# ucla-vision/xivo

Measured on AMD Instinct MI355X. Metric: EKF updates/sec (state dim 250, 80 feats) @1 GPU; % MFMA roofline, higher is better.
Workload: dtype f64; 1 GPU; MH gating + UpdateJosephForm: state dim 250, 80 features (M=160), XIVO row sparsity, P/H/inn/R resident in HBM; filters_per_gpu=16384, global_batch=16384, parallelism=replicas x1 (no collective), pipeline=sparse-H (row-pair compressed H, whitened in-solve Joseph form), hand_over=dense H -> row-pair compressed rows every step, inside the timed region, route=sparse_in_solve, not_spd_filters=0

## Files before the change

### include/xivo_hip.h

```cpp
#ifndef XIVO_HIP_H_
#define XIVO_HIP_H_

#include <stddef.h>

#ifdef __cplusplus
extern "C" {
#endif

typedef struct xivo_hip_ctx xivo_hip_ctx;

enum {
  XIVO_HIP_OK = 0,
  XIVO_HIP_ERR_INVALID = -1,
  XIVO_HIP_ERR_HIP = -2,
  XIVO_HIP_ERR_NOT_SPD = -3,
  XIVO_HIP_ERR_NOMEM = -4,
  XIVO_HIP_ERR_UNSUPPORTED = -5,
  XIVO_HIP_ERR_FULL = -6
};

enum {
  XIVO_HIP_FLAG_NONE = 0u,
  XIVO_HIP_FLAG_FIX_GROUP_BLOCK = 1u,
  XIVO_HIP_FLAG_PROFILE = 2u,
// ... 29 lines not shown
  double Rbc[9], Tbc[3];
  double Vsb[3], bg[3], ba[3];
  double Rsg[9];
} xivo_pose_in;

typedef struct {
  double Rsb[9], Tsb[3];
} xivo_group_in;

typedef struct {
  double x[3];
  double xp[2];
  int ref_sind;
  int sind;
} xivo_feat_in;

#define XIVO_OOS_MAX_OBS 16
typedef struct {
  double Xs[3];
  int n_obs;
  int group_sind[XIVO_OOS_MAX_OBS];
  double xp[XIVO_OOS_MAX_OBS][2];
} xivo_oos_in;

int xivo_hip_create(xivo_hip_ctx** out, int device, int N, int M_max, int batch_max, unsigned flags);
void xivo_hip_destroy(xivo_hip_ctx* ctx);
const char* xivo_hip_strerror(int status);
int xivo_hip_sync(xivo_hip_ctx* ctx);
int xivo_hip_device_count(void);
int xivo_hip_device_numa_node(int device);
int xivo_hip_set_flags(xivo_hip_ctx* ctx, unsigned flags);

int xivo_hip_upload_P(xivo_hip_ctx* ctx, int b0, int nb, const double* P, long stride, int ld);
int xivo_hip_download_P(xivo_hip_ctx* ctx, int b0, int nb, double* P, long stride, int ld);
int xivo_hip_snapshot_P(xivo_hip_ctx* ctx);
int xivo_hip_restore_P(xivo_hip_ctx* ctx);
int xivo_hip_p_zero_rc(xivo_hip_ctx* ctx, int b, int off, int len);
int xivo_hip_p_copy_rc(xivo_hip_ctx* ctx, int b, int dst, int src, int len);
int xivo_hip_p_set_block3(xivo_hip_ctx* ctx, int b, int off, const double* P3);
int xivo_hip_p_diag(xivo_hip_ctx* ctx, int b, double* diag_out);

int xivo_hip_set_measurements(xivo_hip_ctx* ctx, int b0, int nb, int M,
                              const double* H, long strideH, int ldh,
                              const double* inn, long strideInn,
                              const double* diagR, long strideR);
int xivo_hip_set_measurements_device(xivo_hip_ctx* ctx, int b0, int nb, int M,
                                     const double* dH, long strideH, int ldh,
                                     const double* dInn, long strideInn,
                                     const double* dR, long strideR);
int xivo_hip_update_joseph(xivo_hip_ctx* ctx, int B);
int xivo_hip_get_err(xivo_hip_ctx* ctx, int b0, int nb, double* err, long stride);
int xivo_hip_get_status(xivo_hip_ctx* ctx, int b0, int nb, int* status);
int xivo_hip_get_ldlt_used(xivo_hip_ctx* ctx, int b0, int nb, int* used);
#define XIVO_HIP_HOST_P_RESIDENT 1u
#define XIVO_HIP_HOST_KEEP_P 2u
int xivo_hip_update_joseph_host(xivo_hip_ctx* ctx, int b, int M, const double* H, int ldh, const double* inn,
                                const double* diagR, double* P, int ldp, double* err_out, unsigned mode);
int xivo_hip_selftest_fused_tiles(int column_blocks, int* per_simd);
int xivo_hip_selftest_fused_shape(int Mp, int Np, int pw, char* label, int n);
int xivo_hip_selftest_host_compress(const double* H, int ldh, int M, int N, int pairs_clear, int* idx, double* val, int* nc, int* pw);
#define XIVO_HIP_LAUNCH_GATE 0
#define XIVO_HIP_LAUNCH_OOS_COMPRESS 1
#define XIVO_HIP_LAUNCH_PROP_TAIL 2
int xivo_hip_selftest_glevel_launch(int kind, int a, int b, int c, char* label, int n);
int xivo_hip_selftest_ctx_allocs(xivo_hip_ctx* ctx, int* live, unsigned long long* bytes);
int xivo_hip_mh_gate_dense(xivo_hip_ctx* ctx, int B, int F, double R, double mh_thresh,
                           double mh_mult, int min_inliers,
                           unsigned char* inlier_mask_out, double* mh_dist_out);

int xivo_hip_update_dense_gated(xivo_hip_ctx* ctx, int B, int F, double R, double mh_thresh,
                                double mh_mult, int min_inliers);
int xivo_hip_get_gate(xivo_hip_ctx* ctx, int B, int F, unsigned char* inlier_mask_out, double* mh_dist_out);

int xivo_hip_set_layout(xivo_hip_ctx* ctx, const xivo_layout* layout, const xivo_cam* cam);
int xivo_hip_set_scene(xivo_hip_ctx* ctx, int b0, int nb, int F,
                       const xivo_pose_in* poses, const xivo_group_in* groups ,
                       const xivo_feat_in* feats );
int xivo_hip_jacobians_instate(xivo_hip_ctx* ctx, int B);
int xivo_hip_get_jacobians(xivo_hip_ctx* ctx, int b0, int nb, double* J2x21, double* inn2);
typedef struct {
  int td;
  int Cg;
  int cam_begin;
  int cam_dim;
} xivo_calib_layout;
typedef struct {
  double gyro[3];
  double Cg[9];
  double td;
  double Ca[9];
  double intr[9];
} xivo_calib_in;
int xivo_hip_set_calib(xivo_hip_ctx* ctx, const xivo_calib_layout* layout);
int xivo_hip_set_calib_state(xivo_hip_ctx* ctx, int b0, int nb, const xivo_calib_in* calib );
int xivo_hip_get_calib_state(xivo_hip_ctx* ctx, int b0, int nb, xivo_calib_in* calib_out );
int xivo_hip_set_calib_gyro(xivo_hip_ctx* ctx, int b0, int nb, const double* gyro3);
int xivo_hip_get_jacobians_calib(xivo_hip_ctx* ctx, int b0, int nb, double* Jc2x22);
int xivo_hip_mh_gate(xivo_hip_ctx* ctx, int B, double R, double mh_thresh, double mh_mult,
                     int min_inliers, unsigned char* inlier_mask_out, double* mh_dist_out);
int xivo_hip_stack(xivo_hip_ctx* ctx, int B, double R);
int xivo_hip_oos_project(xivo_hip_ctx* ctx, int b0, int nb, int n_oos, const xivo_oos_in* feats,
                         double Roos, int* rows_out);
#define XIVO_HIP_OOS_WHOLE_BUFFER 1u
int xivo_hip_oos_project_ex(xivo_hip_ctx* ctx, int b0, int nb, int n_oos, const xivo_oos_in* feats,
                            double Roos, int* rows_out, unsigned options);
typedef struct {
// ... 190 lines not shown
```

### xivo_amd/csrc/capi_update.hip

```cpp
#include <algorithm>

#include "capi_internal.h"

using namespace xivo_hip;
using namespace xivo_hip::capi;

namespace {

enum UpdateRoute : int { ROUTE_FUSED = 0, ROUTE_SPARSE_IN_SOLVE, ROUTE_SPARSE_WHITENED, ROUTE_SPARSE_SYMMETRIC, ROUTE_SPARSE_TAIL,
                         ROUTE_DENSE_ASCODED, ROUTE_DENSE_WHITENED, ROUTE_DENSE_SYMMETRIC, ROUTE_COUNT };
static const char* kRouteNames[ROUTE_COUNT] = {"fused", "sparse_in_solve", "sparse_whitened", "sparse_symmetric", "sparse_tail",
                                               "dense_ascoded", "dense_whitened", "dense_symmetric"};
struct UpdatePlan {
  int route;
  bool sparse;
  bool in_solve;
  bool latency;
  bool stream8;
  bool f32_whitened;
};

static UpdatePlan plan_update(const xivo_hip_ctx* c, int b0, int B, bool gate) {
  const StagedRows& r = c->rows;
  const int Np = c->Np, Mp = r.rows_padded();
// ... 514 lines not shown
int xivo_hip_update_dense_gated(xivo_hip_ctx* c, int B, int F, double R, double mh_thresh, double mh_mult,
                                int min_inliers) {
  if (c && hipSetDevice(c->device) != hipSuccess) return XIVO_HIP_ERR_HIP;
  if (!c || B <= 0 || B > c->Bmax || c->rows.rows_padded() <= 0 || F <= 0 || 2 * F > c->rows.rows()) return XIVO_HIP_ERR_INVALID;
  int rc = ensure_gate_buffers(c, F);
  if (rc) return rc;
  GateParams gp{F, R, mh_thresh, mh_mult, min_inliers};
  return update_chunks(c, B, F > min_inliers ? &gp : nullptr);
}

int xivo_hip_last_path(xivo_hip_ctx* c) { return c ? c->last_path : -1; }
int xivo_hip_last_route(xivo_hip_ctx* c) { return c ? c->last_route : -1; }
const char* xivo_hip_route_name(int route) { return route >= 0 && route < ROUTE_COUNT ? kRouteNames[route] : ""; }

double xivo_hip_stage_bytes(xivo_hip_ctx* c, int stage) {
  return (c && stage >= 0 && stage < ST_COUNT) ? c->stage_bytes[stage] : 0.0;
}

const char* xivo_hip_stage_kernel(xivo_hip_ctx* c, int stage) {
  return (c && stage >= 0 && stage < ST_COUNT) ? c->stage_kernel[stage] : "";
}

int xivo_hip_get_gate(xivo_hip_ctx* c, int B, int F, unsigned char* mask_out, double* dist_out) {
  if (c && hipSetDevice(c->device) != hipSuccess) return XIVO_HIP_ERR_HIP;
  if (!c || B <= 0 || B > c->Bmax || F <= 0 || !c->mask) return XIVO_HIP_ERR_INVALID;
  const bool strided = c->rows.gate_layout() == GateLayout::strided;
  const size_t ld = strided ? (size_t)c->Fmax : (size_t)F;
  if (strided && F != c->F) return XIVO_HIP_ERR_INVALID;
  if (mask_out) { int rc = d2h_rows(c, mask_out, F, c->mask, ld, F, B); if (rc) return rc; }
  if (dist_out) {
    int rc = d2h_rows(c, dist_out, F * sizeof(double), c->dist, ld * sizeof(double), F * sizeof(double), B);
    if (rc) return rc;
  }
  return XIVO_HIP_OK;
}

int xivo_hip_get_err(xivo_hip_ctx* c, int b0, int nb, double* err, long stride) {
  if (c && hipSetDevice(c->device) != hipSuccess) return XIVO_HIP_ERR_HIP;
  if (bad_range(c, b0, nb) || !err || stride < c->N) return XIVO_HIP_ERR_INVALID;
  if (nb == 0) return XIVO_HIP_OK;
  return d2h_rows(c, err, (size_t)stride * sizeof(double), c->err.from(b0).p, (size_t)c->err.stride * sizeof(double),
                  (size_t)c->N * sizeof(double), nb);
}

int xivo_hip_get_ldlt_used(xivo_hip_ctx* c, int b0, int nb, int* used) {
  if (c && hipSetDevice(c->device) != hipSuccess) return XIVO_HIP_ERR_HIP;
  if (bad_range(c, b0, nb) || !used) return XIVO_HIP_ERR_INVALID;
  if (nb == 0) return XIVO_HIP_OK;
  HIP_TRY(hipMemcpyAsync(used, c->ldlt_used + b0, (size_t)nb * sizeof(int), hipMemcpyDeviceToHost, c->stream));
  HIP_TRY(hipStreamSynchronize(c->stream));
  return XIVO_HIP_OK;
}

int xivo_hip_get_status(xivo_hip_ctx* c, int b0, int nb, int* status) {
  if (c && hipSetDevice(c->device) != hipSuccess) return XIVO_HIP_ERR_HIP;
  if (bad_range(c, b0, nb) || !status) return XIVO_HIP_ERR_INVALID;
  if (nb == 0) return XIVO_HIP_OK;
  HIP_TRY(hipMemcpyAsync(status, c->status + b0, (size_t)nb * sizeof(int), hipMemcpyDeviceToHost, c->stream));
  HIP_TRY(hipStreamSynchronize(c->stream));
  for (int i = 0; i < nb; ++i) if (status[i]) return XIVO_HIP_ERR_NOT_SPD;
  return XIVO_HIP_OK;
}

int xivo_hip_selftest_fused_tiles(int column_blocks, int* per_simd) { return fused_tiles_selftest(column_blocks, per_simd); }
int xivo_hip_selftest_fused_shape(int Mp, int Np, int pw, char* label, int n) {
  return fused_shape_selftest(Mp, Np, pw, label, n > 0 ? (size_t)n : 0);
}

int xivo_hip_selftest_host_compress(const double* H, int ldh, int M, int N, int pairs_clear, int* idx, double* val, int* nc, int* pw) {
  if (!H || !idx || !val || !nc || !pw || M <= 0 || N <= 0 || ldh < M || 2 * pairs_clear < M) return XIVO_HIP_ERR_INVALID;
  xivo_hip_ctx::HostCompressScratch sc;
  return host_compress(sc, H, ldh, M, N, pairs_clear, idx, val, nc, pw);
}

int xivo_hip_update_joseph_host(xivo_hip_ctx* c, int b, int M, const double* H, int ldh, const double* inn,
                                const double* diagR, double* P, int ldp, double* err_out, unsigned mode) {
  if (c && hipSetDevice(c->device) != hipSuccess) return XIVO_HIP_ERR_HIP;
  const bool p_up = !(mode & XIVO_HIP_HOST_P_RESIDENT), p_down = !(mode & XIVO_HIP_HOST_KEEP_P);
  if (bad_range(c, b, 1) || !H || !inn || !diagR || !err_out || M <= 0 || M > c->Mmax || ldh < M ||
      ((p_up || p_down) && (!P || ldp < c->N)))
    return XIVO_HIP_ERR_INVALID;
  const int N = c->N, Np = c->Np, pairs_clear = c->Mpmax / 2;
  auto al = [](size_t x) { return (x + 63) & ~(size_t)63; };
  const size_t o_idx = 0, o_val = al(o_idx + (size_t)pairs_clear * ELL_W * sizeof(int)),
               o_inn = al(o_val + (size_t)pairs_clear * ELL_W * 2 * sizeof(double)), o_R = al(o_inn + (size_t)c->Mpmax * sizeof(double)),
               o_flags = al(o_R + (size_t)c->Mpmax * sizeof(double)), o_Pin = al(o_flags + 4 * sizeof(int)),
               o_Pout = al(o_Pin + (size_t)N * N * sizeof(double)), o_err = al(o_Pout + (size_t)N * N * sizeof(double)),
               o_st = al(o_err + (size_t)N * sizeof(double)), total = al(o_st + 4 * sizeof(int));
  if (!c->pin_h) {
    if (hipHostMalloc(reinterpret_cast<void**>(&c->pin_h), total, hipHostMallocMapped) != hipSuccess) { c->pin_h = nullptr; (void)hipGetLastError(); return XIVO_HIP_ERR_NOMEM; }
    if (hipHostGetDevicePointer(reinterpret_cast<void**>(&c->pin_d), c->pin_h, 0) != hipSuccess || !c->pin_d) {
      hipHostFree(c->pin_h); c->pin_h = nullptr; c->pin_d = nullptr; (void)hipGetLastError(); return XIVO_HIP_ERR_HIP;
    }
  }
  int nc = 0, pw = 0, over = 1;
  const bool want_ell = !(c->flags & XIVO_HIP_FLAG_DENSE_H) && meas_compress_fits(c->Mpmax, Np);
  if (want_ell)
    over = host_compress(c->hc, H, ldh, M, N, pairs_clear, reinterpret_cast<int*>(c->pin_h + o_idx),
                         reinterpret_cast<double*>(c->pin_h + o_val), &nc, &pw);
  if (over) {
    int rc = XIVO_HIP_OK;
    if (p_up) rc = xivo_hip_upload_P(c, b, 1, P, (long)ldp * N, ldp);
    if (!rc) rc = xivo_hip_set_measurements(c, b, 1, M, H, (long)ldh * N, ldh, inn, M, diagR, M);
    if (!rc) rc = update_joseph_range(c, b, 1);
    if (rc) return rc;
    int st = 0;
// ... 68 lines not shown
```

### xivo_amd/csrc/chol_f64.hip

```cpp
#include <stdlib.h>
#include <stdio.h>

#include "mfma_util.h"
#include "chol_device.h"
#include "gate_device.h"

namespace xivo_hip {

namespace {


__global__ __launch_bounds__(64, 4) void chol_f64_kernel(CholArgs g) {
  const int filt = blockIdx.x;
  if (filt >= g.batch) return;
  double* S = g.S + (long)filt * g.strideS;
  double* invD = g.invD + (long)filt * g.strideInvD;
  const long ld = g.lds;
  const int nb = g.Mp / 16;
  const int lane = threadIdx.x;
  const int li = lane & 15, lg = lane >> 4;

  __shared__ double sInv[2][256];
  int bad = 0;

  for (int j = 0; j < nb; ++j) {
    {
      d4 acc0 = d4{0.0, 0.0, 0.0, 0.0}, acc1 = d4{0.0, 0.0, 0.0, 0.0};
      for (int k = 0; k < j; ++k) {
        const double a0 = S[(16 * j + li) + (long)(16 * k + 0 + lg) * ld];
        const double a1 = S[(16 * j + li) + (long)(16 * k + 4 + lg) * ld];
        const double a2 = S[(16 * j + li) + (long)(16 * k + 8 + lg) * ld];
        const double a3 = S[(16 * j + li) + (long)(16 * k + 12 + lg) * ld];
        acc0 = mfma(a0, a0, acc0);
        acc1 = mfma(a1, a1, acc1);
        acc0 = mfma(a2, a2, acc0);
        acc1 = mfma(a3, a3, acc1);
      }
      d4 x, y;
#pragma unroll
      for (int r = 0; r < 4; ++r) x[r] = S[(16 * j + li) + (long)(16 * j + lg + 4 * r) * ld] - (acc0[r] + acc1[r]);
      factor_invert_diag(x, y, bad, 16 * j, li, lg);
#pragma unroll
      for (int r = 0; r < 4; ++r) {
        const int c = lg + 4 * r;
        if (c <= li) {
          S[(16 * j + li) + (long)(16 * j + c) * ld] = x[r];
          S[(16 * j + c) + (long)(16 * j + li) * ld] = x[r];
        }
        sInv[0][c + li * 16] = y[r];
        sInv[1][li + c * 16] = y[r];
      }
    }
    __syncthreads();
    for (int e = lane; e < 512; e += 64) invD[(long)j * 512 + e] = (&sInv[0][0])[e];

    for (int i = j + 1; i < nb; i += 2) {
      const bool two = (i + 1 < nb);
      const int i2 = two ? i + 1 : i;
      d4 accA = d4{0.0, 0.0, 0.0, 0.0}, accB = d4{0.0, 0.0, 0.0, 0.0};
      d4 accA1 = d4{0.0, 0.0, 0.0, 0.0}, accB1 = d4{0.0, 0.0, 0.0, 0.0};
      for (int k = 0; k < j; ++k) {
#pragma unroll
        for (int s = 0; s < 4; ++s) {
          const long col = (long)(16 * k + 4 * s + lg) * ld;
          const double a = S[(16 * j + li) + col];
          const double b1 = S[(16 * i + li) + col];
          const double b2 = S[(16 * i2 + li) + col];
          if (s & 1) { accA1 = mfma(a, b1, accA1); accB1 = mfma(a, b2, accB1); }
          else { accA = mfma(a, b1, accA); accB = mfma(a, b2, accB); }
        }
      }
      d4 rhsA, rhsB;
#pragma unroll
      for (int r = 0; r < 4; ++r) {
        rhsA[r] = S[(16 * i + li) + (long)(16 * j + lg + 4 * r) * ld] - (accA[r] + accA1[r]);
        rhsB[r] = S[(16 * i2 + li) + (long)(16 * j + lg + 4 * r) * ld] - (accB[r] + accB1[r]);
      }
      d4 outA = d4{0.0, 0.0, 0.0, 0.0}, outB = d4{0.0, 0.0, 0.0, 0.0};
#pragma unroll
      for (int s = 0; s < 4; ++s) {
        const double iv = sInv[0][li + (4 * s + lg) * 16];
        outA = mfma(iv, rhsA[s], outA);
        outB = mfma(iv, rhsB[s], outB);
      }
#pragma unroll
      for (int r = 0; r < 4; ++r) {
        S[(16 * i + li) + (long)(16 * j + lg + 4 * r) * ld] = outA[r];
        S[(16 * j + lg + 4 * r) + (long)(16 * i + li) * ld] = outA[r];
        if (two) {
          S[(16 * i2 + li) + (long)(16 * j + lg + 4 * r) * ld] = outB[r];
          S[(16 * j + lg + 4 * r) + (long)(16 * i2 + li) * ld] = outB[r];
        }
      }
    }
    __syncthreads();
  }
  if (lane == 0) g.status[filt] = bad;
}


template <int NB, int MINB, bool PRE, bool UPFRONT, int NW = 4, bool GATE = false>
__global__ __launch_bounds__(64 * NW, MINB) void chol_reg_f64_kernel(CholArgs g, int mirror, CholGateArgs gt) {
  constexpr int RW = (NB + NW - 1) / NW;
  const int filt = blockIdx.x;
  if (filt >= g.batch) return;
  double* S = g.S + (long)filt * g.strideS;
  double* invD = g.invD + (long)filt * g.strideInvD;
  const long ld = g.lds;
  const int nb = g.Mp / 16;
  const int tid = threadIdx.x, lane = tid & 63, wave = __builtin_amdgcn_readfirstlane(tid >> 6);
  const int li = lane & 15, lg = lane >> 4;

  __shared__ double sInv[2][256];
  __shared__ __attribute__((aligned(16))) double sRow[(NB - 1) * 256];
  __shared__ int sBad;
  if (tid == 0) sBad = 0;
  __shared__ unsigned char sRej[GATE ? 16 * NB : 1];
  if constexpr (GATE) {
    static_assert(NW == 4 && !UPFRONT, "the gate rides in the many-factors instantiations");
    double* sdist = sRow;
    const int F = gt.F;
    double* inn = gt.inn + (long)filt * gt.strideInn;
    double* dr = gt.diagR + (long)filt * gt.strideR;
    const double* sd = gt.Sdiag + (long)filt * gt.strideSdiag;
    for (int f = tid; f < F; f += 64 * NW) {
      const double s00 = sd[4 * f] - dr[2 * f] + gt.R;
      const double s10 = sd[4 * f + 2];
      const double s11 = sd[4 * f + 3] - dr[2 * f + 1] + gt.R;
      sdist[f] = mh_dist_2x2(s00, s10, s11, inn[2 * f], inn[2 * f + 1]);
    }
    for (int m = tid; m < 16 * NB; m += 64 * NW) sRej[m] = 0;
    __syncthreads();
    if (wave == 0) {
      const double th = relax_threshold(sdist, F, gt.thresh, gt.mult, gt.min_inliers, lane);
      if (lane == 0) sdist[F] = th;
    }
    __syncthreads();
    const double th = sdist[F];
    for (int f = tid; f < F; f += 64 * NW) {
      const bool in = sdist[f] < th;
      gt.mask[(long)filt * F + f] = in ? 1 : 0;
      gt.dist[(long)filt * F + f] = sdist[f];
      if (!in) {
        sRej[2 * f] = 1; sRej[2 * f + 1] = 1;
        inn[2 * f] = 0.0; inn[2 * f + 1] = 0.0;
        dr[2 * f] = 1.0; dr[2 * f + 1] = 1.0;
        double* val = gt.ellval + (long)filt * gt.strideVal + (long)f * gt.ell_w * 2;
        for (int t = 0; t < 2 * gt.ell_w; ++t) val[t] = 0.0;
      }
    }
    __syncthreads();
    double* PHT = gt.PHT + (long)filt * gt.stridePHT;
    for (int f = 0; f < F; ++f) {
      if (!sRej[2 * f]) continue;
      for (int n = tid; n < gt.Np; n += 64 * NW) { PHT[n + (long)(2 * f) * gt.ldpht] = 0.0; PHT[n + (long)(2 * f + 1) * gt.ldpht] = 0.0; }
    }
    __syncthreads();
  }
  auto gated = [&](double v, int row, int col) -> double {
    if constexpr (GATE) return (sRej[row] | sRej[col]) ? (row == col ? 1.0 : 0.0) : v;
    else return v;
  };

  d4 L[RW][NB];
  d4 sdiag[RW];
#pragma unroll
  for (int ii = 0; ii < RW; ++ii) {
    const int jd = wave + NW * ii;
    if (NW == 4 && jd < nb) {
#pragma unroll
      for (int r = 0; r < 4; ++r) sdiag[ii][r] = gated(S[(16 * jd + li) + (long)(16 * jd + lg + 4 * r) * ld], 16 * jd + li, 16 * jd + lg + 4 * r);
    }
  }

  if (UPFRONT) {
#pragma unroll
    for (int ii = 0; ii < RW; ++ii) {
      const int i = wave + NW * ii;
#pragma unroll
      for (int k = 0; k < NB; ++k) {
        if (k < NW * ii + NW - 1 && k < i && i < nb) {
#pragma unroll
          for (int r = 0; r < 4; ++r) L[ii][k][r] = S[(16 * i + li) + (long)(16 * k + lg + 4 * r) * ld];
        }
      }
    }
  }
  d4 pre0 = d4{0.0, 0.0, 0.0, 0.0}, pre1 = d4{0.0, 0.0, 0.0, 0.0};
  static_for<NB>([&](auto jc) {
    constexpr int j = decltype(jc)::value;
    if (j < nb) {
    constexpr int owner = j % NW, jj = j / NW;
    d4 sreg[RW];
#pragma unroll
    for (int ii = 0; ii < RW; ++ii) {
      const int i = wave + NW * ii;
      if (!UPFRONT && NW * ii + NW - 1 > j && i > j && i < nb) {
#pragma unroll
        for (int r = 0; r < 4; ++r) sreg[ii][r] = gated(S[(16 * i + li) + (long)(16 * j + lg + 4 * r) * ld], 16 * i + li, 16 * j + lg + 4 * r);
      }
    }
    d4 x;
    if (NW != 4 && wave == owner) {
#pragma unroll
      for (int r = 0; r < 4; ++r) sdiag[jj][r] = S[(16 * j + li) + (long)(16 * j + lg + 4 * r) * ld];
    }
    if (wave == owner) {
      d4 acc0 = d4{0.0, 0.0, 0.0, 0.0}, acc1 = d4{0.0, 0.0, 0.0, 0.0};
      if (PRE) { acc0 = pre0; acc1 = pre1; }
#pragma unroll
      for (int k = (PRE && j > 0) ? j - 1 : 0; k < j; ++k) {
        const d4 a = L[jj][k];
        acc0 = mfma(a[0], a[0], acc0);
        acc1 = mfma(a[1], a[1], acc1);
        acc0 = mfma(a[2], a[2], acc0);
        acc1 = mfma(a[3], a[3], acc1);
      }
#pragma unroll
      for (int r = 0; r < 4; ++r) x[r] = sdiag[jj][r] - (acc0[r] + acc1[r]);
    }
    if constexpr (PRE && j + 1 < NB) if (j + 1 < nb && wave == ((j + 1) % NW)) {
      pre0 = d4{0.0, 0.0, 0.0, 0.0}; pre1 = d4{0.0, 0.0, 0.0, 0.0};
#pragma unroll
      for (int k = 0; k < j; ++k) {
        const d4 a = L[(j + 1) / NW][k];
        pre0 = mfma(a[0], a[0], pre0);
        pre1 = mfma(a[1], a[1], pre1);
        pre0 = mfma(a[2], a[2], pre0);
        pre1 = mfma(a[3], a[3], pre1);
      }
    }
    if (wave == owner) {
      int bad = 0;
      d4 y;
      factor_invert_diag(x, y, bad, 16 * j, li, lg);
#pragma unroll
      for (int r = 0; r < 4; ++r) {
        const int c = lg + 4 * r;
        if (c <= li) {
          S[(16 * j + li) + (long)(16 * j + c) * ld] = x[r];
          S[(16 * j + c) + (long)(16 * j + li) * ld] = x[r];
        }
        sInv[0][c + li * 16] = y[r];
        sInv[1][li + c * 16] = y[r];
      }
      if (bad && lane == 0 && sBad == 0) sBad = bad;
#pragma unroll
      for (int k = 0; k < j; ++k) *reinterpret_cast<d4*>(&sRow[(k * 64 + lane) * 4]) = L[jj][k];
    }
    lds_barrier();
    if (wave == owner)
      for (int e = lane; e < 512; e += 64) invD[(long)j * 512 + e] = (&sInv[0][0])[e];
#pragma unroll
    for (int ii = 0; ii < RW; ++ii) {
      const int i = wave + NW * ii;
      if (NW * ii + NW - 1 > j && i > j && i < nb) {
        d4 accA = d4{0.0, 0.0, 0.0, 0.0}, accB = d4{0.0, 0.0, 0.0, 0.0};
#pragma unroll
        for (int k = 0; k < j; ++k) {
          if (k < NW * ii + NW - 1) {
            const d4 a = *reinterpret_cast<const d4*>(&sRow[(k * 64 + lane) * 4]);
            const d4 bb = L[ii][k];
            accA = mfma(a[0], bb[0], accA);
            accB = mfma(a[1], bb[1], accB);
            accA = mfma(a[2], bb[2], accA);
            accB = mfma(a[3], bb[3], accB);
          }
        }
        d4 rhs;
#pragma unroll
        for (int r = 0; r < 4; ++r) rhs[r] = (UPFRONT ? L[ii][j][r] : sreg[ii][r]) - (accA[r] + accB[r]);
        d4 out = d4{0.0, 0.0, 0.0, 0.0};
#pragma unroll
        for (int s4 = 0; s4 < 4; ++s4) out = mfma(sInv[0][li + (4 * s4 + lg) * 16], rhs[s4], out);
        L[ii][j] = out;
#pragma unroll
        for (int r = 0; r < 4; ++r) {
          S[(16 * i + li) + (long)(16 * j + lg + 4 * r) * ld] = out[r];
          if (mirror) S[(16 * j + lg + 4 * r) + (long)(16 * i + li) * ld] = out[r];
        }
      }
    }
    lds_barrier();
    }
  });
  if (tid == 0) g.status[filt] = sBad;
}

}

static bool chol_one_wave_forced() { static const bool on = getenv("XIVO_HIP_CHOL_WAVE") != nullptr; return on; }
static int chol_reg_mode(int batch) { return batch >= 512 ? 0 : 2; }

bool chol_gate_supported(int Mp, int batch) {
  return !chol_one_wave_forced() && Mp / 16 <= 12 && chol_reg_mode(batch) == 0;
}

int launch_chol_f64(const CholArgs& g, hipStream_t stream, const CholGateArgs* gate) {
  if (g.batch <= 0) return 0;
  const CholGateArgs nogate{};
  if (gate && !chol_gate_supported(g.Mp, g.batch)) return (int)hipErrorInvalidValue;
  const int nb = g.Mp / 16;
  if (!chol_one_wave_forced() && nb <= 12) {
    const int mirror = (nb > 10 || g.latency) ? 1 : 0;
    const bool many = g.batch >= 512;
    const int mode = chol_reg_mode(g.batch);
    if (gate && mode != 0) return (int)hipErrorInvalidValue;
#define CHOL_REG_LAUNCH(NB_, MINB_)                                                                                                     \
  do {                                                                                                                                  \
    if (mode == 0 && gate) hipLaunchKernelGGL((chol_reg_f64_kernel<NB_, MINB_, false, false, 4, true>), dim3(g.batch), dim3(256), 0, stream, g, mirror, *gate); \
    else if (mode == 0) hipLaunchKernelGGL((chol_reg_f64_kernel<NB_, MINB_, false, false>), dim3(g.batch), dim3(256), 0, stream, g, mirror, nogate);   \
    else hipLaunchKernelGGL((chol_reg_f64_kernel<NB_, MINB_, true, true>), dim3(g.batch), dim3(256), 0, stream, g, mirror, nogate);             \
  } while (0)
    if (nb <= 4) CHOL_REG_LAUNCH(4, 2);
    else if (nb <= 8) CHOL_REG_LAUNCH(8, 2);
    else if (nb <= 10 && many) CHOL_REG_LAUNCH(10, 3);
    else if (nb <= 10) CHOL_REG_LAUNCH(10, 2);
    else if (many) CHOL_REG_LAUNCH(12, 3);
    else CHOL_REG_LAUNCH(12, 2);
#undef CHOL_REG_LAUNCH
    return (int)hipGetLastError();
  }
  if (gate) return (int)hipErrorInvalidValue;
  if (!chol_one_wave_forced() && nb > 12 && nb <= 19) {
    const int mirror = 1;
    const bool pre = g.batch < 512;
    if (nb <= 16) {
      if (pre) hipLaunchKernelGGL((chol_reg_f64_kernel<16, 1, true, false, 8>), dim3(g.batch), dim3(512), 0, stream, g, mirror, nogate);
      else hipLaunchKernelGGL((chol_reg_f64_kernel<16, 1, false, false, 8>), dim3(g.batch), dim3(512), 0, stream, g, mirror, nogate);
    } else {
      if (pre) hipLaunchKernelGGL((chol_reg_f64_kernel<19, 1, true, false, 8>), dim3(g.batch), dim3(512), 0, stream, g, mirror, nogate);
      else hipLaunchKernelGGL((chol_reg_f64_kernel<19, 1, false, false, 8>), dim3(g.batch), dim3(512), 0, stream, g, mirror, nogate);
    }
    return (int)hipGetLastError();
  }
  hipLaunchKernelGGL(chol_f64_kernel, dim3(g.batch), dim3(64), 0, stream, g);
  return (int)hipGetLastError();
}
// ... 11 lines not shown
```

### xivo_amd/lib.py

```python
import ctypes as C
import os
import numpy as np

_HERE = os.path.dirname(os.path.abspath(__file__))
OOS_MAX_OBS = 16

FLAG_FIX_GROUP_BLOCK = 1
FLAG_PROFILE = 2
FLAG_DENSE_H = 64
FLAG_SYMMETRIC_FORM = 256
FLAG_STANDALONE_TAIL = 512
FLAG_NO_LDLT_FALLBACK = 4096
FLAG_FP32_WHITENED = 16384
FLAG_THROUGHPUT_ROUTE = 8192
FLAG_INVDEPTH = 32768
OOS_WHOLE_BUFFER = 1
FLAG_MULTI_KERNEL = 65536
CAM_PINHOLE, CAM_ATAN, CAM_RADTAN, CAM_EQUI = 0, 1, 2, 3


class XivoHipError(RuntimeError):
    def __init__(self, status, msg):
        super().__init__(f"xivo_hip status {status}: {msg}")
        self.status = status
# ... 96 lines not shown
    "xivo_hip_update_dense_gated": [C.c_void_p, C.c_int, C.c_int, C.c_double, C.c_double, C.c_double, C.c_int],
    "xivo_hip_get_gate": [C.c_void_p, C.c_int, C.c_int, C.c_void_p, C.c_void_p],
    "xivo_hip_set_layout": [C.c_void_p, C.POINTER(Layout), C.POINTER(Cam)],
    "xivo_hip_set_scene": [C.c_void_p, C.c_int, C.c_int, C.c_int, C.c_void_p, C.c_void_p, C.c_void_p],
    "xivo_hip_jacobians_instate": [C.c_void_p, C.c_int],
    "xivo_hip_get_jacobians": [C.c_void_p, C.c_int, C.c_int, C.c_void_p, C.c_void_p],
    "xivo_hip_mh_gate": [C.c_void_p, C.c_int, C.c_double, C.c_double, C.c_double, C.c_int, C.c_void_p,
                         C.c_void_p],
    "xivo_hip_stack": [C.c_void_p, C.c_int, C.c_double],
    "xivo_hip_oos_project": [C.c_void_p, C.c_int, C.c_int, C.c_int, C.c_void_p, C.c_double, C.c_void_p],
    "xivo_hip_oos_project_ex": [C.c_void_p, C.c_int, C.c_int, C.c_int, C.c_void_p, C.c_double, C.c_void_p, C.c_uint],
    "xivo_hip_close_loop_stack": [C.c_void_p, C.c_int, C.c_int, C.c_int, C.c_void_p, C.c_double],
    "xivo_hip_compress_oos": [C.c_void_p, C.c_int, C.c_double, C.c_void_p],
    "xivo_hip_one_point_ransac": [C.c_void_p, C.c_int, C.c_double, C.c_double, C.c_double, C.c_void_p, C.c_void_p, C.c_void_p,
                                  C.c_void_p, C.c_void_p],
    "xivo_hip_filter_update": [C.c_void_p, C.c_int, C.c_double, C.c_double, C.c_double, C.c_int, C.c_int],
    "xivo_hip_last_path": [C.c_void_p],
    "xivo_hip_last_route": [C.c_void_p],
    "xivo_hip_stage_kernel": [C.c_void_p, C.c_int],
    "xivo_hip_stage_bytes": [C.c_void_p, C.c_int],
    "xivo_hip_absorb_error": [C.c_void_p, C.c_int],
    "xivo_hip_propagate": [C.c_void_p, C.c_int, C.c_int, C.c_int, C.c_void_p, C.c_void_p],
    "xivo_hip_givens": [C.c_void_p, C.c_int, C.c_int, C.c_int, C.c_int, C.c_void_p, C.c_void_p, C.c_void_p, C.c_int,
                        C.c_void_p],
    "xivo_hip_qr": [C.c_void_p, C.c_int, C.c_int, C.c_int, C.c_void_p, C.c_void_p, C.c_int, C.c_void_p],
    "xivo_hip_subfilter_update": [C.c_void_p, C.c_int, C.c_int, C.c_int, C.c_void_p, C.c_void_p],
    "xivo_hip_candidate_order": [C.c_void_p, C.c_int, C.c_int, C.c_int, C.c_int, C.c_void_p, C.c_void_p, C.c_void_p],
    "xivo_hip_pool_config": [C.c_void_p, C.c_int, C.c_int, C.c_void_p, C.c_double],
    "xivo_hip_pool_anchor": [C.c_void_p, C.c_int, C.c_int, C.c_void_p],
    "xivo_hip_pool_add": [C.c_void_p, C.c_int, C.c_void_p],
    "xivo_hip_pool_step": [C.c_void_p, C.c_int, C.c_void_p, C.c_int, C.c_void_p, C.c_void_p, C.c_void_p],
    "xivo_hip_pool_get": [C.c_void_p, C.c_int, C.c_int, C.c_void_p, C.c_void_p, C.c_void_p],
    "xivo_hip_triangulate": [C.c_void_p, C.c_int, C.c_void_p, C.c_void_p, C.c_void_p],
    "xivo_hip_pool_triangulation": [C.c_void_p, C.c_void_p],
    "xivo_hip_pool_tri_counts": [C.c_void_p, C.c_int, C.c_int, C.c_void_p, C.c_void_p],
    "xivo_hip_pool_adapt_depth_config": [C.c_void_p, C.c_void_p],
    "xivo_hip_pool_adapt_depth": [C.c_void_p, C.c_int, C.c_void_p],
    "xivo_hip_pool_add_ex": [C.c_void_p, C.c_int, C.c_void_p, C.c_uint],
    "xivo_hip_edit_batch": [C.c_void_p, C.c_int, C.c_int, C.c_void_p],
    "xivo_hip_set_pixels": [C.c_void_p, C.c_int, C.c_int, C.c_int, C.c_void_p],
    "xivo_hip_get_scene": [C.c_void_p, C.c_int, C.c_int, C.c_void_p, C.c_void_p, C.c_void_p],
    "xivo_hip_get_H": [C.c_void_p, C.c_int, C.POINTER(C.c_int), C.c_void_p, C.c_int, C.c_void_p, C.c_void_p],
    "xivo_hip_propagate_cov": [C.c_void_p, C.c_int, C.c_int, C.c_int, C.c_void_p, C.c_void_p],
    "xivo_hip_dev_alloc": [C.c_void_p, C.c_size_t, C.POINTER(C.c_void_p)],
    "xivo_hip_dev_free": [C.c_void_p, C.c_void_p],
    "xivo_hip_dev_upload": [C.c_void_p, C.c_void_p, C.c_void_p, C.c_size_t, C.c_size_t],
    "xivo_hip_timer_begin": [C.c_void_p],
    "xivo_hip_timer_end": [C.c_void_p, C.POINTER(C.c_float)],
    "xivo_hip_profile_reset": [C.c_void_p],
    "xivo_hip_profile_get": [C.c_void_p, C.POINTER(C.c_int), C.POINTER(C.c_char_p), C.POINTER(C.c_float),
                             C.POINTER(C.c_int), C.POINTER(C.c_double)],
    "xivo_hip_bench_mfma_peak": [C.c_void_p, C.POINTER(C.c_double)],
    "xivo_hip_get_ldlt_used": [C.c_void_p, C.c_int, C.c_int, C.c_void_p],
    "xivo_hip_update_joseph_host": [C.c_void_p, C.c_int, C.c_int, C.c_void_p, C.c_int, C.c_void_p, C.c_void_p, C.c_void_p, C.c_int,
                                    C.c_void_p, C.c_uint],
    "xivo_hip_set_calib": [C.c_void_p, C.c_void_p],
    "xivo_hip_set_calib_state": [C.c_void_p, C.c_int, C.c_int, C.c_void_p],
    "xivo_hip_get_jacobians_calib": [C.c_void_p, C.c_int, C.c_int, C.c_void_p],
    "xivo_hip_get_calib_state": [C.c_void_p, C.c_int, C.c_int, C.c_void_p],
    "xivo_hip_set_calib_gyro": [C.c_void_p, C.c_int, C.c_int, C.c_void_p],
    "xivo_hip_propagate_calib": [C.c_void_p, C.c_int, C.c_int, C.c_int, C.c_void_p, C.c_void_p, C.c_void_p],
    "xivo_hip_selftest_fused_tiles": [C.c_int, C.c_void_p],
    "xivo_hip_selftest_fused_shape": [C.c_int, C.c_int, C.c_int, C.c_void_p, C.c_int],
    "xivo_hip_selftest_host_compress": [C.c_void_p, C.c_int, C.c_int, C.c_int, C.c_int, C.c_void_p, C.c_void_p, C.c_void_p, C.c_void_p],
    "xivo_hip_selftest_glevel_launch": [C.c_int, C.c_int, C.c_int, C.c_int, C.c_void_p, C.c_int],
    "xivo_hip_selftest_ctx_allocs": [C.c_void_p, C.c_void_p, C.c_void_p],
    "xivo_hip_traj_config": [C.c_void_p, C.c_void_p],
    "xivo_hip_traj_record": [C.c_void_p, C.c_int, C.c_longlong, C.c_void_p],
    "xivo_hip_traj_count": [C.c_void_p],
    "xivo_hip_traj_reset": [C.c_void_p],
    "xivo_hip_traj_read": [C.c_void_p, C.c_int, C.c_int, C.c_int, C.c_int, C.c_void_p, C.c_void_p, C.c_void_p],
    "xivo_hip_traj_nees": [C.c_void_p, C.c_int, C.c_int, C.c_int, C.c_int, C.c_void_p, C.c_void_p, C.c_void_p, C.c_void_p,
                           C.c_void_p],
}
HOST_P_RESIDENT, HOST_KEEP_P = 1, 2


def tri_options(method, zmin=0.05, zmax=5.0, max_theta_thresh=0.1 * np.pi / 180, beta_thresh=0.25 * np.pi / 180):
    o = np.zeros(1, dtype=tri_opts_dtype)
    o["struct_size"] = tri_opts_dtype.itemsize
    o["method"] = TRI_METHODS[method] if isinstance(method, str) else int(method)
    o["zmin"], o["zmax"], o["max_theta_thresh"], o["beta_thresh"] = zmin, zmax, max_theta_thresh, beta_thresh
    return o


class CalibLayout(C.Structure):
    _fields_ = [("td", C.c_int), ("Cg", C.c_int), ("cam_begin", C.c_int), ("cam_dim", C.c_int)]


calib_dtype = np.dtype([("gyro", "f8", 3), ("Cg", "f8", 9), ("td", "f8"), ("Ca", "f8", 9), ("intr", "f8", 9)])
assert calib_dtype.itemsize == 248


def cam_intr(cam):
    d = list(cam.get("d", [])) + [0.0] * 5
    return np.array([cam["fx"], cam["fy"], cam["cx"], cam["cy"]] + d[:5], dtype=np.float64)
ALL_SYMBOLS = sorted(list(_SIGS) + ["xivo_hip_destroy", "xivo_hip_strerror", "xivo_hip_gemm_tile", "xivo_hip_device_count",
                                        "xivo_hip_device_numa_node", "xivo_hip_route_name"])


def load_library():
    global _LIB
    if _LIB is not None:
        return _LIB
    path = lib_path()
    if not os.path.exists(path):
# ... 172 lines not shown
        calib = np.ascontiguousarray(calib, dtype=calib_dtype)
        self._check(self.lib.xivo_hip_set_calib_state(self.h, b0, calib.shape[0], _ptr(calib)))

    def set_calib_gyro(self, gyro, b0=0):
        gyro = np.ascontiguousarray(gyro, dtype=np.float64).reshape(-1, 3)
        self._check(self.lib.xivo_hip_set_calib_gyro(self.h, b0, gyro.shape[0], _ptr(gyro)))

    def get_calib_state(self, b0=0, nb=None):
        nb = self.batch - b0 if nb is None else nb
        out = np.zeros(nb, dtype=calib_dtype)
        self._check(self.lib.xivo_hip_get_calib_state(self.h, b0, nb, _ptr(out)))
        return out

    def get_jacobians_calib(self, b0=0, nb=None, F=None):
        nb = self.batch - b0 if nb is None else nb
        out = np.empty((nb, F, 2, 22))
        self._check(self.lib.xivo_hip_get_jacobians_calib(self.h, b0, nb, _ptr(out)))
        return out

    def update_joseph_host(self, H, inn, diagR, P_cm, b=0, mode=0, check=True):
        H = np.asarray(H, dtype=np.float64)
        M, N = H.shape
        assert N == self.N, (N, self.N)
        assert P_cm is None or (P_cm.dtype == np.float64 and P_cm.flags["F_CONTIGUOUS"] and P_cm.shape == (N, N))
        Hc = _f64(H.T)
        inn = _f64(inn); dR = _f64(diagR)
        err = np.empty(self.N)
        rc = self.lib.xivo_hip_update_joseph_host(self.h, b, M, _ptr(Hc), M, _ptr(inn), _ptr(dR),
                                                  None if P_cm is None else _ptr(P_cm), self.N, _ptr(err), mode)
        if check:
            self._check(rc)
        return err, rc

    def get_err(self, b0=0, nb=None):
        nb = self.batch - b0 if nb is None else nb
        out = np.empty((nb, self.N))
        self._check(self.lib.xivo_hip_get_err(self.h, b0, nb, _ptr(out), self.N))
        return out

    def get_status(self, b0=0, nb=None, check=True):
        nb = self.batch - b0 if nb is None else nb
        out = np.zeros(nb, dtype=np.int32)
        rc = self.lib.xivo_hip_get_status(self.h, b0, nb, _ptr(out))
        if check:
            self._check(rc)
        return out

    def get_ldlt_used(self, b0=0, nb=None):
        nb = self.batch - b0 if nb is None else nb
        out = np.zeros(nb, dtype=np.int32)
        self._check(self.lib.xivo_hip_get_ldlt_used(self.h, b0, nb, _ptr(out)))
        return out

    def mh_gate_dense(self, F, R, thresh, mult, min_inliers, B=None):
        B = self.batch if B is None else B
        mask = np.zeros((B, F), dtype=np.uint8)
        dist = np.zeros((B, F))
        self._check(self.lib.xivo_hip_mh_gate_dense(self.h, B, F, R, thresh, mult, min_inliers, _ptr(mask),
                                                    _ptr(dist)))
        return mask.astype(bool), dist

    def update_dense_gated(self, F, R, thresh, mult, min_inliers, B=None):
        self._check(self.lib.xivo_hip_update_dense_gated(self.h, self.batch if B is None else B, F, R, thresh, mult,
                                                         min_inliers))

    def get_gate(self, F, B=None):
        B = self.batch if B is None else B
        mask = np.zeros((B, F), dtype=np.uint8)
        dist = np.zeros((B, F))
        self._check(self.lib.xivo_hip_get_gate(self.h, B, F, _ptr(mask), _ptr(dist)))
        return mask.astype(bool), dist

    def set_layout(self, N, group_begin, n_groups, feature_begin, n_features, cam):
        lay = Layout(N, group_begin, n_groups, feature_begin, n_features)
        self.layout = lay
        c = Cam()
        c.model, c.rows, c.cols = cam["model"], cam.get("rows", 480), cam.get("cols", 640)
        c.fx, c.fy, c.cx, c.cy = cam["fx"], cam["fy"], cam["cx"], cam["cy"]
        d = list(cam.get("d", [])) + [0.0] * 5
        for i in range(5):
            c.d[i] = d[i]
        self._check(self.lib.xivo_hip_set_layout(self.h, C.byref(lay), C.byref(c)))

    def set_scene(self, poses, groups, feats, b0=0):
        poses = np.ascontiguousarray(poses, dtype=pose_dtype)
        groups = np.ascontiguousarray(groups, dtype=group_dtype)
        feats = np.ascontiguousarray(feats, dtype=feat_dtype)
        nb, F = feats.shape
        self.F = F
        self._check(self.lib.xivo_hip_set_scene(self.h, b0, nb, F, _ptr(poses), _ptr(groups), _ptr(feats)))

    def jacobians_instate(self, B=None):
        self._check(self.lib.xivo_hip_jacobians_instate(self.h, self.batch if B is None else B))

    def get_jacobians(self, b0=0, nb=None):
        nb = self.batch - b0 if nb is None else nb
        J = np.empty((nb, self.F, 2, 21))
        inn = np.empty((nb, self.F, 2))
        self._check(self.lib.xivo_hip_get_jacobians(self.h, b0, nb, _ptr(J), _ptr(inn)))
        return J, inn

    def mh_gate(self, R, thresh, mult, min_inliers, B=None, want=True):
        B = self.batch if B is None else B
        if not want:
            self._check(self.lib.xivo_hip_mh_gate(self.h, B, R, thresh, mult, min_inliers, None, None))
            return None
# ... 307 lines not shown
```

Baseline: 954,400 updates/s.

## Prefetch next Cholesky block column during triangular solve and defer stores

In the register-blocked Cholesky kernel (4-wave, non-upfront, non-PRE instantiations), the next block column of S is loaded into registers while the current column's triangular solve is in progress. Stores of the solved blocks are deferred until after all solves, and gating moves from load time to the point of use. Diagonal blocks now load before the gate phase, and the gate's __syncthreads become lds_barrier. It also adds optional compile-time timing instrumentation and a host API to read back the factor. The aim is to hide global-load latency behind MFMA work, at the cost of more register pressure and possible spills.

```diff
diff --git a/include/xivo_hip.h b/include/xivo_hip.h
--- a/include/xivo_hip.h
+++ b/include/xivo_hip.h
@@ -105,6 +105,7 @@
 int xivo_hip_get_err(xivo_hip_ctx* ctx, int b0, int nb, double* err, long stride);
 int xivo_hip_get_status(xivo_hip_ctx* ctx, int b0, int nb, int* status);
 int xivo_hip_get_ldlt_used(xivo_hip_ctx* ctx, int b0, int nb, int* used);
+int xivo_hip_get_factor(xivo_hip_ctx* ctx, int b0, int nb, double* L, double* inv_diag);
 #define XIVO_HIP_HOST_P_RESIDENT 1u
 #define XIVO_HIP_HOST_KEEP_P 2u
 int xivo_hip_update_joseph_host(xivo_hip_ctx* ctx, int b, int M, const double* H, int ldh, const double* inn,
diff --git a/xivo_amd/csrc/capi_update.hip b/xivo_amd/csrc/capi_update.hip
--- a/xivo_amd/csrc/capi_update.hip
+++ b/xivo_amd/csrc/capi_update.hip
@@ -590,6 +590,23 @@
   return XIVO_HIP_OK;
 }
 
+int xivo_hip_get_factor(xivo_hip_ctx* c, int b0, int nb, double* L, double* inv_diag) {
+  if (c && hipSetDevice(c->device) != hipSuccess) return XIVO_HIP_ERR_HIP;
+  if (bad_range(c, b0, nb) || (!L && !inv_diag)) return XIVO_HIP_ERR_INVALID;
+  const int Mp = c->rows.rows_padded();
+  if (nb == 0 || Mp <= 0) return XIVO_HIP_OK;
+  const BatchMat S = c->S.from(b0);
+  const BatchVec invD = c->invD.from(b0);
+  const size_t inv_n = (size_t)(Mp / 16) * 512;
+  for (int b = 0; b < nb; ++b) {
+    if (L) HIP_TRY(hipMemcpy2DAsync(L + (size_t)b * Mp * Mp, (size_t)Mp * sizeof(double), S.p + (long)b * S.stride, (size_t)S.ld * sizeof(double),
+                                    (size_t)Mp * sizeof(double), Mp, hipMemcpyDeviceToHost, c->stream));
+    if (inv_diag) HIP_TRY(hipMemcpyAsync(inv_diag + (size_t)b * inv_n, invD.p + (long)b * invD.stride, inv_n * sizeof(double), hipMemcpyDeviceToHost, c->stream));
+  }
+  HIP_TRY(hipStreamSynchronize(c->stream));
+  return XIVO_HIP_OK;
+}
+
 int xivo_hip_get_status(xivo_hip_ctx* c, int b0, int nb, int* status) {
   if (c && hipSetDevice(c->device) != hipSuccess) return XIVO_HIP_ERR_HIP;
   if (bad_range(c, b0, nb) || !status) return XIVO_HIP_ERR_INVALID;
diff --git a/xivo_amd/csrc/chol_f64.hip b/xivo_amd/csrc/chol_f64.hip
--- a/xivo_amd/csrc/chol_f64.hip
+++ b/xivo_amd/csrc/chol_f64.hip
@@ -4,6 +4,26 @@
 #include "mfma_util.h"
 #include "chol_device.h"
 #include "gate_device.h"
+
+#ifndef XIVO_CHOL_TRACE
+#define XIVO_CHOL_TRACE 0
+#endif
+#if XIVO_CHOL_TRACE
+__device__ unsigned long long xivo_chol_trace_buf[256 * 4 * 13 * 8];
+#define CTR_ON (GATE && NB <= 12 && (blockIdx.x & 63) == 0)
+#define CTR(col, slot) do { if (CTR_ON && lane == 0) sTr[(wave * 13 + (col)) * 8 + (slot)] = __builtin_amdgcn_s_memtime(); } while (0)
+#define CTR_ADD(col, slot, dt) do { if (CTR_ON && lane == 0) sTr[(wave * 13 + (col)) * 8 + (slot)] += (dt); } while (0)
+#define CTR_NOW() __builtin_amdgcn_s_memtime()
+#define CTR_ARRIVED(v) asm volatile("" :: "v"(v))
+extern "C" int xivo_hip_debug_read_chol_trace(unsigned long long* out, int n) {
+  return (int)hipMemcpyFromSymbol(out, HIP_SYMBOL(xivo_chol_trace_buf), (size_t)n * sizeof(unsigned long long));
+}
+#else
+#define CTR(col, slot) do {} while (0)
+#define CTR_ADD(col, slot, dt) do {} while (0)
+#define CTR_NOW() 0ull
+#define CTR_ARRIVED(v) do {} while (0)
+#endif
 
 namespace xivo_hip {
 
@@ -98,10 +118,23 @@
   if (lane == 0) g.status[filt] = bad;
 }
 
+template <int J, int NW, int RW>
+__device__ __forceinline__ void request_block_column(d4 (&dst)[RW], const double* S, long ld, int nb, int wave, int li, int lg) {
+#pragma unroll
+  for (int ii = 0; ii < RW; ++ii) {
+    const int i = wave + NW * ii;
+    if (NW * ii + NW - 1 > J && i > J && i < nb) {
+#pragma unroll
+      for (int r = 0; r < 4; ++r) dst[ii][r] = S[(16 * i + li) + (long)(16 * J + lg + 4 * r) * ld];
+    }
+  }
+}
+
 
 template <int NB, int MINB, bool PRE, bool UPFRONT, int NW = 4, bool GATE = false>
 __global__ __launch_bounds__(64 * NW, MINB) void chol_reg_f64_kernel(CholArgs g, int mirror, CholGateArgs gt) {
   constexpr int RW = (NB + NW - 1) / NW;
+  constexpr bool AHEAD = NW == 4 && !UPFRONT && !PRE;
   const int filt = blockIdx.x;
   if (filt >= g.batch) return;
   double* S = g.S + (long)filt * g.strideS;
@@ -115,7 +148,23 @@
   __shared__ __attribute__((aligned(16))) double sRow[(NB - 1) * 256];
   __shared__ int sBad;
   if (tid == 0) sBad = 0;
+#if XIVO_CHOL_TRACE
+  __shared__ unsigned long long sTr[4 * 13 * 8];
+  if (CTR_ON) { for (int e = tid; e < 4 * 13 * 8; e += 64 * NW) sTr[e] = 0; __syncthreads(); }
+  CTR(NB, 0);
+#endif
   __shared__ unsigned char sRej[GATE ? 16 * NB : 1];
+  d4 sdiag[RW];
+#pragma unroll
+  for (int ii = 0; ii < RW; ++ii) {
+    const int jd = wave + NW * ii;
+    if (NW == 4 && jd < nb) {
+#pragma unroll
+      for (int r = 0; r < 4; ++r) sdiag[ii][r] = S[(16 * jd + li) + (long)(16 * jd + lg + 4 * r) * ld];
+    }
+  }
+  d4 sreg[RW];
+  if constexpr (AHEAD) request_block_column<0, NW, RW>(sreg, S, ld, nb, wave, li, lg);
   if constexpr (GATE) {
     static_assert(NW == 4 && !UPFRONT, "the gate rides in the many-factors instantiations");
     double* sdist = sRow;
@@ -130,12 +179,12 @@
       sdist[f] = mh_dist_2x2(s00, s10, s11, inn[2 * f], inn[2 * f + 1]);
     }
     for (int m = tid; m < 16 * NB; m += 64 * NW) sRej[m] = 0;
-    __syncthreads();
+    lds_barrier();
     if (wave == 0) {
       const double th = relax_threshold(sdist, F, gt.thresh, gt.mult, gt.min_inliers, lane);
       if (lane == 0) sdist[F] = th;
     }
-    __syncthreads();
+    lds_barrier();
     const double th = sdist[F];
     for (int f = tid; f < F; f += 64 * NW) {
       const bool in = sdist[f] < th;
@@ -149,29 +198,21 @@
         for (int t = 0; t < 2 * gt.ell_w; ++t) val[t] = 0.0;
       }
     }
-    __syncthreads();
+    lds_barrier();
     double* PHT = gt.PHT + (long)filt * gt.stridePHT;
     for (int f = 0; f < F; ++f) {
       if (!sRej[2 * f]) continue;
       for (int n = tid; n < gt.Np; n += 64 * NW) { PHT[n + (long)(2 * f) * gt.ldpht] = 0.0; PHT[n + (long)(2 * f + 1) * gt.ldpht] = 0.0; }
     }
-    __syncthreads();
-  }
+    lds_barrier();
+  }
+  CTR(NB, 1);
   auto gated = [&](double v, int row, int col) -> double {
     if constexpr (GATE) return (sRej[row] | sRej[col]) ? (row == col ? 1.0 : 0.0) : v;
     else return v;
   };
 
   d4 L[RW][NB];
-  d4 sdiag[RW];
-#pragma unroll
-  for (int ii = 0; ii < RW; ++ii) {
-    const int jd = wave + NW * ii;
-    if (NW == 4 && jd < nb) {
-#pragma unroll
-      for (int r = 0; r < 4; ++r) sdiag[ii][r] = gated(S[(16 * jd + li) + (long)(16 * jd + lg + 4 * r) * ld], 16 * jd + li, 16 * jd + lg + 4 * r);
-    }
-  }
 
   if (UPFRONT) {
 #pragma unroll
@@ -191,16 +232,10 @@
     constexpr int j = decltype(jc)::value;
     if (j < nb) {
     constexpr int owner = j % NW, jj = j / NW;
-    d4 sreg[RW];
-#pragma unroll
-    for (int ii = 0; ii < RW; ++ii) {
-      const int i = wave + NW * ii;
-      if (!UPFRONT && NW * ii + NW - 1 > j && i > j && i < nb) {
-#pragma unroll
-        for (int r = 0; r < 4; ++r) sreg[ii][r] = gated(S[(16 * i + li) + (long)(16 * j + lg + 4 * r) * ld], 16 * i + li, 16 * j + lg + 4 * r);
-      }
-    }
+    CTR(j, 0);
+    if constexpr (!AHEAD && !UPFRONT) request_block_column<j, NW, RW>(sreg, S, ld, nb, wave, li, lg);
     d4 x;
+    CTR(j, 1);
     if (NW != 4 && wave == owner) {
 #pragma unroll
       for (int r = 0; r < 4; ++r) sdiag[jj][r] = S[(16 * j + li) + (long)(16 * j + lg + 4 * r) * ld];
@@ -217,7 +252,7 @@
         acc1 = mfma(a[3], a[3], acc1);
       }
 #pragma unroll
-      for (int r = 0; r < 4; ++r) x[r] = sdiag[jj][r] - (acc0[r] + acc1[r]);
+      for (int r = 0; r < 4; ++r) x[r] = gated(sdiag[jj][r], 16 * j + li, 16 * j + lg + 4 * r) - (acc0[r] + acc1[r]);
     }
     if constexpr (PRE && j + 1 < NB) if (j + 1 < nb && wave == ((j + 1) % NW)) {
       pre0 = d4{0.0, 0.0, 0.0, 0.0}; pre1 = d4{0.0, 0.0, 0.0, 0.0};
@@ -248,13 +283,36 @@
 #pragma unroll
       for (int k = 0; k < j; ++k) *reinterpret_cast<d4*>(&sRow[(k * 64 + lane) * 4]) = L[jj][k];
     }
-    lds_barrier();
+    CTR(j, 2);
+#if XIVO_CHOL_TRACE
+#pragma unroll
+    for (int ii = 0; ii < RW; ++ii) {
+      const int i = wave + NW * ii;
+      if (!UPFRONT && NW * ii + NW - 1 > j && i > j && i < nb) {
+#pragma unroll
+        for (int r = 0; r < 4; ++r) CTR_ARRIVED(sreg[ii][r]);
+      }
+    }
+#endif
+    CTR(j, 3);
+    lds_barrier();
+    CTR(j, 4);
     if (wave == owner)
       for (int e = lane; e < 512; e += 64) invD[(long)j * 512 + e] = (&sInv[0][0])[e];
+    auto store_block = [&](int ii, int i) {
+      const unsigned long long ts0 = CTR_NOW();
+#pragma unroll
+      for (int r = 0; r < 4; ++r) {
+        S[(16 * i + li) + (long)(16 * j + lg + 4 * r) * ld] = L[ii][j][r];
+        if (mirror) S[(16 * j + lg + 4 * r) + (long)(16 * i + li) * ld] = L[ii][j][r];
+      }
+      CTR_ADD(j, 6, CTR_NOW() - ts0);
+    };
 #pragma unroll
     for (int ii = 0; ii < RW; ++ii) {
       const int i = wave + NW * ii;
       if (NW * ii + NW - 1 > j && i > j && i < nb) {
+        const unsigned long long tc0 = CTR_NOW();
         d4 accA = d4{0.0, 0.0, 0.0, 0.0}, accB = d4{0.0, 0.0, 0.0, 0.0};
 #pragma unroll
         for (int k = 0; k < j; ++k) {
@@ -269,21 +327,38 @@
         }
         d4 rhs;
 #pragma unroll
-        for (int r = 0; r < 4; ++r) rhs[r] = (UPFRONT ? L[ii][j][r] : sreg[ii][r]) - (accA[r] + accB[r]);
+        for (int r = 0; r < 4; ++r) rhs[r] = gated(UPFRONT ? L[ii][j][r] : sreg[ii][r], 16 * i + li, 16 * j + lg + 4 * r) - (accA[r] + accB[r]);
+        if constexpr (AHEAD && j + 1 < NB) if (NW * ii + NW - 1 > j + 1 && i > j + 1) {
+#pragma unroll
+          for (int r = 0; r < 4; ++r) sreg[ii][r] = S[(16 * i + li) + (long)(16 * (j + 1) + lg + 4 * r) * ld];
+        }
         d4 out = d4{0.0, 0.0, 0.0, 0.0};
 #pragma unroll
         for (int s4 = 0; s4 < 4; ++s4) out = mfma(sInv[0][li + (4 * s4 + lg) * 16], rhs[s4], out);
         L[ii][j] = out;
-#pragma unroll
-        for (int r = 0; r < 4; ++r) {
-          S[(16 * i + li) + (long)(16 * j + lg + 4 * r) * ld] = out[r];
-          if (mirror) S[(16 * j + lg + 4 * r) + (long)(16 * i + li) * ld] = out[r];
-        }
-      }
-    }
-    lds_barrier();
+        CTR_ARRIVED(out[3]);
+        CTR_ADD(j, 5, CTR_NOW() - tc0);
+        if constexpr (!AHEAD) store_block(ii, i);
+      }
+    }
+    if constexpr (AHEAD) {
+#pragma unroll
+      for (int ii = 0; ii < RW; ++ii) {
+        const int i = wave + NW * ii;
+        if (NW * ii + NW - 1 > j && i > j && i < nb) store_block(ii, i);
+      }
+    }
+    lds_barrier();
+    CTR(j, 7);
     }
   });
+#if XIVO_CHOL_TRACE
+  CTR(NB, 2);
+  if (CTR_ON && (blockIdx.x >> 6) < 256) {
+    __syncthreads();
+    for (int e = tid; e < 4 * 13 * 8; e += 64 * NW) xivo_chol_trace_buf[(blockIdx.x >> 6) * (4 * 13 * 8) + e] = sTr[e];
+  }
+#endif
   if (tid == 0) g.status[filt] = sBad;
 }
 
diff --git a/xivo_amd/lib.py b/xivo_amd/lib.py
--- a/xivo_amd/lib.py
+++ b/xivo_amd/lib.py
@@ -172,6 +172,7 @@
                              C.POINTER(C.c_int), C.POINTER(C.c_double)],
     "xivo_hip_bench_mfma_peak": [C.c_void_p, C.POINTER(C.c_double)],
     "xivo_hip_get_ldlt_used": [C.c_void_p, C.c_int, C.c_int, C.c_void_p],
+    "xivo_hip_get_factor": [C.c_void_p, C.c_int, C.c_int, C.c_void_p, C.c_void_p],
     "xivo_hip_update_joseph_host": [C.c_void_p, C.c_int, C.c_int, C.c_void_p, C.c_int, C.c_void_p, C.c_void_p, C.c_void_p, C.c_int,
                                     C.c_void_p, C.c_uint],
     "xivo_hip_set_calib": [C.c_void_p, C.c_void_p],
@@ -450,6 +451,13 @@
         self._check(self.lib.xivo_hip_get_ldlt_used(self.h, b0, nb, _ptr(out)))
         return out
 
+    def get_factor(self, M, b0=0, nb=None):
+        nb = self.batch - b0 if nb is None else nb
+        Mp = (M + 15) // 16 * 16
+        Lcm = np.zeros((nb, Mp, Mp)); inv = np.zeros((nb, Mp // 16, 2, 16, 16))
+        self._check(self.lib.xivo_hip_get_factor(self.h, b0, nb, _ptr(Lcm), _ptr(inv)))
+        return np.tril(np.transpose(Lcm, (0, 2, 1))), inv
+
     def mh_gate_dense(self, F, R, thresh, mult, min_inliers, B=None):
         B = self.batch if B is None else B
         mask = np.zeros((B, F), dtype=np.uint8)
```

Measured after the change: 953,300 updates/s. About the same (-0.1%).
